# galatolofederico/clip-glass

Measured on AMD Instinct MI355X. Metric: candidate latents scored/sec (GAN→CLIP fitness), StyleGAN2_ffhq_d pop=64, higher is better.
Workload: dtype f16; 1 GPU; StyleGAN2_ffhq_d: StyleGAN2 config-f 1024px G+D + CLIP ViT-B/32, pop=64 per GPU, batch_size=4, n_obj=2; pop_per_gpu=64, global_pop=64, batch_size=4, parallelism=population-shard x1, device=AMD Radeon Graphics (gfx950:sramecc+:xnack-), 256 CUs, hbm_gib=288

## Files before the change

### clip_glass_amd/csrc/kernels.h

```cpp
#pragma once
#include "common.h"

#include <string>
#include <vector>

const char* launch_conv_direct(const ConvParams& p, hipStream_t st);
const char* launch_gemm_direct(const GemmParams& p, hipStream_t st);
const char* launch_conv_tiled(const ConvParams& p, hipStream_t st);
const char* launch_gemm_tiled(const GemmParams& p, hipStream_t st);
const char* launch_conv_stream(const ConvParams& p, hipStream_t st);
const char* launch_conv_gemm(const ConvParams& p, half_t* ws_a, long long cap_a, float* ws_c, long long cap_c, hipStream_t st);
bool conv_stream_applies(const ConvParams& p);
const char* launch_conv_glds(const ConvParams& p, hipStream_t st);
const char* launch_conv_wreg(const ConvParams& p, hipStream_t st);
bool conv_wreg_supported(int Cin, int Cout, int H, int W);
const char* launch_conv_s2(const ConvParams& p, hipStream_t st, bool force = false);
const char* launch_conv_down(const half_t* h, const half_t* xs, const half_t* w1, const half_t* ws, const float* b1, half_t* y,
                             int B, int R, int Cin, int Cout, hipStream_t st);
bool conv_down_supported(int R, int Cin, int Cout);
const char* launch_dblock0(const float* rgb_y, const float* rgb_w, const float* rgb_b, const half_t* w0, const float* b0, const half_t* w1,
                           const half_t* ws, const float* b1, half_t* y, int B, int R, int Cin, int Cout, hipStream_t st, int y_planar8 = 0);
bool dblock0_supported(int R, int Cin, int Cout);
const char* launch_upconv_fused(const ConvParams& p, hipStream_t st);

void launch_pixelnorm(const float* z, float* out, int P, int L, float eps, hipStream_t st);
void launch_dense01_finish(const float* part, int S, long long slab, const float* bias0, const float* w1, const float* b1, float* out, int P, int N,
                           hipStream_t st);
void launch_dense_splitk(const float* x, int ldx, int P, int K, const float* wt, int N, const float* bias, float* out, int ldo,
                         int mode, hipStream_t st);
void launch_dense(const float* x, int ldx, int P, int K, const float* wt, int N, const float* bias,
                  float* out, int ldo, int in_sq, int mode, const float* eps_row, int eps_stride,
                  hipStream_t st);
bool launch_mapping_fused(const float* z, float* out, int P, int L, float eps, const float* const* wt, const float* const* b, int n_layers,
                          hipStream_t st);
struct DenseDesc {
    const float* x; int ldx; int K; const float* wt; int N; const float* bias; float* out; int ldo;
    const float* eps_row; int eps_stride;
};
void launch_dense_multi(const DenseDesc* d_desc, int n_desc, int max_N, int P, int in_sq, int mode, hipStream_t st);
void launch_style_norm(float* s, int ld, int P, int n_layers, const int* d_off, const int* d_len,
                       float* smax, float* eps_row, float eps, hipStream_t st);
void launch_modulate_weights(const half_t* w, long long elems, int Cin, int Cout, const float* sn, int sn_stride,
                              const float* dscale, int ds_stride, int P, half_t* wm, hipStream_t st);
void launch_noise(float* out, int n_mb, int hw, uint32_t layer, uint32_t mb0, uint32_t generation,
                  uint64_t seed, hipStream_t st);

void launch_trgb_tables(const float* wrgb, const float* sn, int sn_stride, const float* smax, int smax_stride, int B, int NT,
                        half_t* tab, hipStream_t st);
void launch_trgb_finish(const float* part, int ntn, int B, int R, const float* bias, const float* yprev, float* yout, hipStream_t st);
bool launch_torgb(const half_t* x, int B, int H, int W, int C, const float* wrgb, const float* bias,
                  const float* sn, int sn_stride, const float* smax, int smax_stride,
                  const float* yprev, float* yout, hipStream_t st);
void launch_finalize_image(const float* y, float* img, long long n, hipStream_t st);
void launch_resize_patches(const float* y, int B, int R, int clip_res, int ps, int ld, half_t* patches,
                           hipStream_t st);
#define GLASS_RESIZE_MAX_TAPS 32
#define PREPROCESS_TY 8
#define PREPROCESS_RB 8
#define PREPROCESS_MAX_R 1024
struct ResizeTaps {
    std::vector<int> start, count;
    std::vector<float> taps;
    std::vector<float> table;
    int max_count = 0, nr = 0, ts = 0;
    size_t lds_bytes = 0;
};
struct ResizeTapsDev {
    const float* table = nullptr;
    int n4 = 0, ts = 0;
    size_t lds_bytes = 0;
};
bool build_resize_taps(int R, int S, int mode, ResizeTaps& t, std::string& why);
void launch_preprocess_patches(const float* y, int B, int R, int clip_res, int ps, int ld, int resize_mode, int normalize,
                               const ResizeTapsDev& t, half_t* patches, hipStream_t st);
void launch_fromrgb(const float* y, int B, int R, int Cout, const float* w, const float* bias,
                    half_t* out, hipStream_t st);
// ... 78 lines not shown
```

### clip_glass_amd/csrc/ops.hip

```cpp
#include <string.h>

#include <string>
#include <vector>

#include "../../include/glass_ops.h"
#include "engine.h"
#include "kernels.h"

namespace {
struct Dev {
    std::vector<void*> ptrs;
    ~Dev() {
        for (void* p : ptrs) hipFree(p);
    }
    template <typename T>
    T* alloc(size_t n) {
        void* q = nullptr;
        if (hipMalloc(&q, (n ? n : 1) * sizeof(T)) != hipSuccess) return nullptr;
        ptrs.push_back(q);
        return (T*)q;
    }
    half_t* up16(const float* src, size_t n) {
        if (!src) return nullptr;
        std::vector<_Float16> h(n);
// ... 63 lines not shown
        std::vector<_Float16> pk2;
        glass_pack_conv(d->w, d->Cout, d->Cin, 3, d->Cin, pk2);
        p.w_up = dv.up16v(pk2);
    }
    p.sn = dv.up32(d->sn, (size_t)d->B * d->Cin); p.sn_stride = d->Cin;
    p.sn16 = dv.up16(d->sn, (size_t)d->B * d->Cin);
    p.dscale = dv.up32(d->dscale, (size_t)d->B * d->Cout); p.ds_stride = d->Cout;
    p.batch_size = d->batch_size > 0 ? d->batch_size : 1;
    p.noise = dv.up32(d->noise, (size_t)(d->B / p.batch_size) * d->Ho * d->Wo);
    p.noise_strength = d->noise_strength;
    p.bias = dv.up32(d->bias, d->Cout);
    p.act = d->act;
    const size_t nout = (size_t)d->B * d->Ho * d->Wo * d->Cout;
    p.res = dv.up16(d->res, nout);
    p.out_scale = d->out_scale;
    half_t* y = dv.alloc<half_t>(nout);
    p.y = y;
    OPREQ(p.x && p.w && y, "device allocation failed");
    if (d->skip_x) {
        OPREQ(d->skip_w && (d->impl == 2 || d->impl == 5), "fused skip branch: impl 2 / 5 with skip_x and skip_w");
        std::vector<_Float16> pks;
        glass_pack_conv(d->skip_w, d->Cout, d->Cin, 1, d->Cin, pks);
        p.skip_w = dv.up16v(pks);
        p.skip_x = dv.up16(d->skip_x, (size_t)d->B * d->Ho * d->Wo * d->Cin);
    }
    half_t* xs_dev = nullptr;
    const size_t nxs = (size_t)d->B * (d->H / 2) * (d->W / 2) * d->Cin;
    if (d->xs_out) {
        OPREQ(d->impl == 2 || d->impl == 5, "blur-down by-product: impl 2 / 5");
        xs_dev = dv.alloc<half_t>(nxs);
        p.xs_out = xs_dev;
    }
    float* yrgb = nullptr;
    const size_t nrgb = (size_t)d->B * 3 * d->Ho * d->Wo;
    if (d->trgb_yout) {
        OPREQ((d->impl == 4 || d->impl == 2 || d->impl == 5) && d->trgb_w && d->trgb_b && d->trgb_sn && d->trgb_smax,
              "fused toRGB: impl 2 / 4 / 5 and all of w / b / sn / smax");
        p.trgb_w = dv.up32(d->trgb_w, 3 * (size_t)d->Cout); p.trgb_b = dv.up32(d->trgb_b, 3);
        p.trgb_sn = dv.up32(d->trgb_sn, (size_t)d->B * d->Cout); p.trgb_sn_stride = d->Cout;
        p.trgb_smax = dv.up32(d->trgb_smax, d->B); p.trgb_smax_stride = 1;
        p.trgb_yprev = dv.up32(d->trgb_yprev, (size_t)d->B * 3 * (d->Ho / 2) * (d->Wo / 2));
        yrgb = dv.alloc<float>(nrgb);
        p.trgb_yout = yrgb;
        if (d->impl == 4) {
            p.y = nullptr;
        } else {
            half_t* tab = dv.alloc<half_t>((size_t)d->B * 32 * d->Cout);
            launch_trgb_tables(p.trgb_w, p.trgb_sn, p.trgb_sn_stride, p.trgb_smax, p.trgb_smax_stride, d->B, d->Cout, tab, 0);
            p.trgb_tab = tab;
        }
    }
    p.x_planar8 = d->x_planar8;
    p.x_planar32 = d->x_planar32;
    if (d->impl == 1) { if (!launch_conv_direct(p, 0)) { glass_set_error("direct conv: unsupported launch"); return GLASS_ERR_ARG; } }
    else if (d->impl == 3) {
        if (!launch_upconv_fused(p, 0)) { glass_set_error("fused up-conv: unsupported shape"); return GLASS_ERR_ARG; }
    } else if (d->impl == 2) {
        if (!launch_conv_tiled(p, 0)) { glass_set_error("tiled conv: unsupported shape"); return GLASS_ERR_ARG; }
    } else if (d->impl == 4) {
        if (!launch_conv_stream(p, 0)) { glass_set_error("streaming conv: unsupported shape"); return GLASS_ERR_ARG; }
    } else if (d->impl == 6) {
        const long long cap_a = (long long)p.Hc * p.Wc * p.KS * p.KS * p.Cin, cap_c = (long long)p.Hc * p.Wc * p.Neff;
        half_t* wa = dv.alloc<half_t>((size_t)(cap_a * p.B));
        float* wc = dv.alloc<float>((size_t)(cap_c * p.B));
        if (!launch_conv_gemm(p, wa, cap_a, wc, cap_c, 0)) { glass_set_error("im2col + GEMM conv: unsupported shape"); return GLASS_ERR_ARG; }
    } else if (d->impl == 5) {
        if (p.skip_x) {
            if (!launch_conv_s2(p, 0, true)) { glass_set_error("LDS-DMA stride-2 conv: unsupported shape"); return GLASS_ERR_ARG; }
        } else if (!launch_conv_glds(p, 0)) { glass_set_error("LDS-DMA conv: unsupported shape"); return GLASS_ERR_ARG; }
    } else if (!(d->up && launch_upconv_fused(p, 0)) && !launch_conv_stream(p, 0) && !launch_conv_tiled(p, 0) && !launch_conv_direct(p, 0)) {
        glass_set_error("no kernel accepts this convolution");
        return GLASS_ERR_ARG;
    }
    int rc = finish();
    if (rc) return rc;
    if (yrgb) {
        GLASS_HIP(hipMemcpy(d->trgb_yout, yrgb, nrgb * sizeof(float), hipMemcpyDeviceToHost));
        return p.y ? down16(d->y, y, nout) : GLASS_OK;
    }
    if (xs_dev && (rc = down16(d->xs_out, xs_dev, nxs))) return rc;
    return down16(d->y, y, nout);
}

extern "C" int glass_op_gemm(int32_t device, int32_t M, int32_t N, int32_t K, const float* a, const float* w,
                             const float* bias, int32_t mode, int32_t impl, float* out) {
    OPREQ(a && w && out && K % 16 == 0, "bad argument");
    GLASS_HIP(hipSetDevice(device));
    Dev dv;
    GemmParams g;
    memset(&g, 0, sizeof g);
    g.a = dv.up16(a, (size_t)M * K); g.w = dv.up16(w, (size_t)N * K); g.M = M; g.N = N; g.K = K;
    g.bias = dv.up32(bias, N); g.mode = mode; g.ldo = N;
    const size_t n = (size_t)M * N;
    half_t* o16 = nullptr; float* o32 = nullptr;
    if (mode <= 1) { o16 = dv.alloc<half_t>(n); g.out16 = o16; }
    else { o32 = mode == 2 ? dv.up32(out, n) : dv.alloc<float>(n); g.out32 = o32; }
    if (impl == 1) launch_gemm_direct(g, 0);
    else if (impl == 2) {
        if (!launch_gemm_tiled(g, 0)) { glass_set_error("tiled gemm: unsupported shape"); return GLASS_ERR_ARG; }
    } else if (!launch_gemm_tiled(g, 0)) launch_gemm_direct(g, 0);
    int rc = finish();
    if (rc) return rc;
    if (o16) return down16(out, o16, n);
    GLASS_HIP(hipMemcpy(out, o32, n * sizeof(float), hipMemcpyDeviceToHost));
    return GLASS_OK;
}

extern "C" int glass_op_dense(int32_t device, int32_t P, int32_t K, int32_t N, const float* x, const float* wt,
                              const float* bias, int32_t in_sq, int32_t mode, const float* eps_row, float* out) {
// ... 462 lines not shown
```

### clip_glass_amd/csrc/upfir.hip

```cpp
#include "common.h"
#include "kernels.h"
#include <algorithm>
#include <mutex>
#include <vector>

#define ROWB 80

struct UpGeo {
    int NTn, ngroups;
    int tiles_x, n_seg, S;
    int NXI, NYI, n_grids;
    int WT;
    unsigned invPX, invPY;
    unsigned inv2PX, inv2PY;
};

namespace {
constexpr int U_PH = 9, U_PW = 33;
constexpr int U_NVB = 9 * 32 * 4, U_NB = (U_NVB + 255) / 256;
constexpr int U_A_BYTES = ((U_PH * U_PW * ROWB + 15) / 16) * 16;
struct UStep {
    static constexpr int RW = 2, MR = 4 * RW, TR = 2 * MR, PH = MR + 1;
    static constexpr int NVA = PH * U_PW * 4, NA = (NVA + 255) / 256;
    static constexpr int A_BYTES = ((PH * U_PW * ROWB + 15) / 16) * 16;
    static constexpr int T_BYTES = TR * 64 * 64;
    static constexpr int STAGE = A_BYTES + 9 * 32 * ROWB;
    static constexpr int R0 = ((T_BYTES > STAGE ? T_BYTES : STAGE) + 1023) / 1024 * 1024;
    static constexpr int OFF_LNZ = R0;
    static constexpr int OFF_HS = OFF_LNZ + TR * 60 * 4;
    static constexpr int LDS = OFF_HS + 256 * 48;
};
constexpr int U_OFF_STY = 46848;
constexpr int U_OFF_DS = U_OFF_STY + 8 * 1024;
constexpr int U_OFF_PS = U_OFF_DS + 8 * 128;
constexpr int U_OFF_BI = U_OFF_PS + 8 * 64;
constexpr int U_OFF_NZ = U_OFF_BI + 128;
static_assert(UStep::LDS == 81664 && 2 * UStep::LDS <= 163840, "two workgroups per CU");
static_assert(U_OFF_NZ + 16 * 60 * 4 <= 65536 && U_OFF_STY >= U_A_BYTES + 9 * 32 * ROWB && UStep::A_BYTES == U_A_BYTES, "constant tables fit behind the staging images");
__device__ __forceinline__ int u_opaque(int v) { asm volatile("" : "+v"(v)); return v; }
__device__ __forceinline__ int u_stage_row(int r) { return (r & ~7) | ((r & 7) >> 1) | ((r & 1) << 2); }
__device__ __forceinline__ int u_tpos(int x) { return (x & 1) * 32 + (x >> 1); }
__device__ __forceinline__ int u_fir_col(int ci) { return ci ^ (((ci >> 2) ^ (ci >> 1)) & 1); }
}

template <bool GRID>
__global__ __launch_bounds__(256, 2) void upfir2_kernel(ConvParams p, UpGeo g) {
    using US = UStep;
    constexpr int RW = US::RW, MR = US::MR, TR = US::TR;
    constexpr int PW = U_PW, NA = US::NA, NVB = U_NVB, NB = U_NB, A_BYTES = US::A_BYTES;
    constexpr int U_OFF_LNZ = US::OFF_LNZ, U_OFF_HS = US::OFF_HS;
    extern __shared__ __attribute__((aligned(16))) char smem[];
    char* As = smem;
    char* Bs = smem + A_BYTES;
    half_t* T = (half_t*)smem;

    const int id = blockIdx.x;
// ... 367 lines not shown
                    const int ltx = oxl + 1 + jx;
                    tr[jx] = (const char*)T + u_tpos(ltx) * 64 + ((cg ^ ((ltx >> 2) & 3)) * 16);
                }
                const long long rowpitch = (long long)p.Wo * (p.y_planar8 ? 8 : p.Cout);
                half_t* yp = p.y_planar8 ? p.y + ((((long long)img0 * 4 * g.NTn + (n0 >> 3) + cg) * p.Ho + ovy0) * p.Wo + ox) * 8
                                          : p.y + (((long long)img0 * p.Ho + ovy0) * p.Wo + ox) * p.Cout + n0 + cg * 8;
                h8 cv[4];
                float cnz;
                auto rdrow = [&](int r, h8 (&v_)[4], float& nz_) {
#pragma unroll
                    for (int jx = 0; jx < 4; ++jx) v_[jx] = *(const h8*)(tr[jx] + r * 4096);
                    nz_ = *(const float*)(smem + U_OFF_LNZ + (r * 60 + oxl) * 4);
                };
                rdrow(0, cv, cnz);
#pragma unroll
                for (int r = 0; r < TR; ++r) {
                    h8 nv[4];
                    float nnz;
                    if (r + 1 < TR) rdrow(r + 1, nv, nnz);
                    __builtin_amdgcn_sched_barrier(0);
                    hs[r & 3] = (cv[1] + cv[2]) * f3 + (cv[0] + cv[3]);
                    const h8 bn = bias8 + (half_t)cnz;
                    h8 v = (hs[(r - 3) & 3] + hs[r & 3]) * fq4 + ((hs[(r - 2) & 3] + hs[(r - 1) & 3]) * ft4 + bn);
                    v = __builtin_elementwise_max(v, v * slope) * kps;
                    if ((step > 0 || r >= 4) && ovy0 + r < p.Ho) *(h8*)yp = v;
                    yp += rowpitch;
                    __builtin_amdgcn_sched_barrier(0);
                    if (r + 1 < TR) {
#pragma unroll
                        for (int jx = 0; jx < 4; ++jx) cv[jx] = nv[jx];
                        cnz = nnz;
                    }
                }
                *(h8*)(hs_slot) = hs[1]; *(h8*)(hs_slot + 16) = hs[2]; *(h8*)(hs_slot + 32) = hs[3];
            }
            if (step + 1 < g.S && Y0 + TR * (step + 1) - 4 < out_rows) {
                const int my0n = my0 + MR;
                const bool plain_n = mx0 >= 1 && my0n >= 1 && my0n + MR - 1 < p.H && mx0 + 31 < p.W;
                load_b(0);
                if (plain && plain_n) {
                    const int dstep = MR * p.W * p.Cin;
#pragma unroll
                    for (int k = 0; k < NA; ++k) a_goff[k] += dstep;
                } else {
                    aim(my0n, 0);
                }
                load_a(0);
                have = true;
            }
        }
    }
}

static unsigned u_inv(int d) { return (unsigned)((0x100000000ULL + (unsigned)d - 1) / (unsigned)d); }

static int upfir2_model_steps(int per_seg, int out_rows, int TR, int slots, int fallback) {
    struct Key { int per_seg, out_rows, slots, S; };
    static std::mutex mu;
    static std::vector<Key> cache;
    std::lock_guard<std::mutex> lk(mu);
    for (const Key& k : cache)
        if (k.per_seg == per_seg && k.out_rows == out_rows && k.slots == slots) return k.S;
    int best = fallback;
    double best_t = 1e30;
    std::vector<double> heap;
    for (int S = 1; S <= 16; ++S) {
        const int R = (TR - 4) + TR * (S - 1);
        if (R > out_rows + TR - 1 && S > 1) break;
        const int n_seg = (out_rows + R - 1) / R;
        if ((long long)per_seg * n_seg < slots) break;
        heap.assign(slots, 0.0);
        auto cmp = [](double a, double b) { return a > b; };
        for (int seg = 0; seg < n_seg; ++seg) {
            int steps = 0;
            for (int st = 0; st < S; ++st) {
                if (seg * R + (st ? TR * st - 4 : 0) >= out_rows) break;
                ++steps;
            }
            for (int w = 0; w < per_seg; ++w) {
                std::pop_heap(heap.begin(), heap.end(), cmp);
                heap.back() += steps + 0.5;
                std::push_heap(heap.begin(), heap.end(), cmp);
            }
        }
        double t = 0;
        for (double v : heap) t = v > t ? v : t;
        if (t < best_t - 1e-9) { best_t = t; best = S; }
    }
    cache.push_back({per_seg, out_rows, slots, best});
    return best;
}

static const char* launch_upfir2(const ConvParams& p, hipStream_t st) {
    if (p.Cin > 512 || p.H < 8 || p.W < 8) return nullptr;
    if ((long long)p.B * p.H * p.W * p.Cin >= (1LL << 31) || 9LL * p.Cout * p.Cin >= (1LL << 31)) return nullptr;
    if (p.x_bstride != (long long)p.H * p.W * p.Cin) return nullptr;
    const bool lean = p.w_bstride && !p.sn16 && !p.dscale;
    if (p.y_planar8 && !lean) return nullptr;
    constexpr int LDS = UStep::LDS, TR = UStep::TR;
    if (!glass_lds_fits(LDS)) return nullptr;
    static DevOnce once;
    once.run([&] {
        (void)hipFuncSetAttribute((const void*)upfir2_kernel<true>, hipFuncAttributeMaxDynamicSharedMemorySize, LDS);
        (void)hipFuncSetAttribute((const void*)upfir2_kernel<false>, hipFuncAttributeMaxDynamicSharedMemorySize, LDS);
    });
    UpGeo g;
    g.NTn = p.Cout / 32;
    if (p.w_bstride) { g.NXI = 1; g.NYI = 1; }
    else {
        const int nxi_max = p.W + 1 >= 11 ? 8 : 3;
        g.NXI = p.B < nxi_max ? p.B : nxi_max;
        g.NYI = (p.B + g.NXI - 1) / g.NXI;
        if (g.NYI > 8) g.NYI = 8;
    }
    g.n_grids = (p.B + g.NXI * g.NYI - 1) / (g.NXI * g.NYI);
    const int PX = p.W + 1, PY = p.H + 1;
    g.tiles_x = (2 * PX * g.NXI - 2 + 59) / 60;
    const int out_rows = 2 * PY * g.NYI - 2;
    int S = 16;
    for (; S > 1; --S) {
        const int R = (TR - 4) + TR * (S - 1);
        const long long wgs = (long long)g.n_grids * g.tiles_x * ((out_rows + R - 1) / R) * g.NTn;
        if (wgs >= (S > 8 ? 5120 : 2048) && R <= out_rows + TR - 1) break;
    }
    if (!lean && S <= 2) S = upfir2_model_steps(g.n_grids * g.tiles_x * g.NTn, out_rows, TR, 2 * glass_cu_count(), S);
    g.S = S;
    const int R = (TR - 4) + TR * (S - 1);
    g.n_seg = (out_rows + R - 1) / R;
    g.WT = g.n_grids * g.n_seg * g.tiles_x;
    int ng = 1;
    if (!p.w_bstride) {
        const long long per_tile = 9LL * 32 * p.Cin * 2;
        while (ng < 8 && g.NTn % (ng * 2) == 0 && (g.NTn / ng) * per_tile > (1200LL << 10)) ng *= 2;
    }
    g.ngroups = ng;
    g.invPX = u_inv(PX); g.invPY = u_inv(PY); g.inv2PX = u_inv(2 * PX); g.inv2PY = u_inv(2 * PY);
    const char* name = lean ? "upfir2_kernel<false>" : "upfir2_kernel<true>";
    if (p.dry_run) return name;
    const int Pp = 8 / ng;
    const int grid = 8 * ((g.WT + Pp - 1) / Pp) * (g.NTn / ng);
    if (lean) hipLaunchKernelGGL((upfir2_kernel<false>), dim3(grid), dim3(256), LDS, st, p, g);
    else hipLaunchKernelGGL((upfir2_kernel<true>), dim3(grid), dim3(256), LDS, st, p, g);
    return name;
}

const char* launch_upconv_fused(const ConvParams& p, hipStream_t st) {
    if (!p.up || !p.w_up || p.y32 || !p.y || p.res || (p.sn && !p.sn16)) return nullptr;
    if (p.Cin % 32 != 0 || p.Cout % 32 != 0 || p.KS != 3) return nullptr;
    if (p.x_planar8 || p.x_planar32) return nullptr;
    return launch_upfir2(p, st);
}
```

### clip_glass_amd/ops.py

```python
import ctypes as C

import numpy as np

from .engine import _check, _f32, _fp, load_library


class ConvDesc(C.Structure):
    _fields_ = [("B", C.c_int32), ("H", C.c_int32), ("W", C.c_int32), ("Cin", C.c_int32), ("Cout", C.c_int32),
                ("KS", C.c_int32), ("stride", C.c_int32), ("pad", C.c_int32), ("up", C.c_int32),
                ("Ho", C.c_int32), ("Wo", C.c_int32), ("broadcast_x", C.c_int32), ("act", C.c_int32),
                ("batch_size", C.c_int32), ("impl", C.c_int32),
                ("noise_strength", C.c_float), ("out_scale", C.c_float),
                ("x", C.POINTER(C.c_float)), ("w", C.POINTER(C.c_float)), ("sn", C.POINTER(C.c_float)),
                ("dscale", C.POINTER(C.c_float)), ("noise", C.POINTER(C.c_float)), ("bias", C.POINTER(C.c_float)),
                ("res", C.POINTER(C.c_float)), ("y", C.POINTER(C.c_float)),
                ("trgb_w", C.POINTER(C.c_float)), ("trgb_b", C.POINTER(C.c_float)), ("trgb_sn", C.POINTER(C.c_float)),
                ("trgb_smax", C.POINTER(C.c_float)), ("trgb_yprev", C.POINTER(C.c_float)),
                ("trgb_yout", C.POINTER(C.c_float)),
                ("skip_x", C.POINTER(C.c_float)), ("skip_w", C.POINTER(C.c_float)), ("xs_out", C.POINTER(C.c_float)),
                ("x_planar8", C.c_int32), ("x_planar32", C.c_int32)]


def to_planar8(a):
    B, H, W, Cc = a.shape
    return np.ascontiguousarray(a.reshape(B, H, W, Cc // 8, 8).transpose(0, 3, 1, 2, 4))


def to_planar32(a):
    B, H, W, Cc = a.shape
    return np.ascontiguousarray(a.reshape(B, H, W, Cc // 32, 32).transpose(0, 3, 1, 2, 4))


def from_planar32(a, B, H, W, Cc):
    return np.ascontiguousarray(a.reshape(B, Cc // 32, H, W, 32).transpose(0, 2, 3, 1, 4)).reshape(B, H, W, Cc)


def from_planar8(a, B, H, W, Cc):
    return np.ascontiguousarray(a.reshape(B, Cc // 8, H, W, 8).transpose(0, 2, 3, 1, 4)).reshape(B, H, W, Cc)


def _opt(a):
    if a is None:
        return None, None
    a = _f32(a)
    return a, _fp(a)


def conv(x, w, *, stride=1, pad=None, up=False, sn=None, dscale=None, noise=None, noise_strength=0.0,
         batch_size=1, bias=None, act=False, res=None, out_scale=1.0, impl=0, broadcast_x=False, B=None, device=0,
         torgb=None, skip=None, xs_out=None, planar_x=False, both=False, planar32_x=False):
    lib = load_library()
    x = _f32(x); w = _f32(w)
    Bx, H, W, Cin = x.shape
    if planar_x:
        x = to_planar8(x)
    if planar32_x:
        x = to_planar32(x)
    B = B if B is not None else Bx
    Cout, _, KS, _ = w.shape
    pad = (KS // 2) if pad is None else pad
    if up:
        Ho, Wo = 2 * H, 2 * W
    else:
        Ho, Wo = (H + 2 * pad - KS) // stride + 1, (W + 2 * pad - KS) // stride + 1
    y = np.empty((B, Ho, Wo, Cout), dtype=np.float32)
    d = ConvDesc()
    d.B, d.H, d.W, d.Cin, d.Cout = B, H, W, Cin, Cout
    d.KS, d.stride, d.pad, d.up, d.Ho, d.Wo = KS, stride, pad, int(up), Ho, Wo
    d.broadcast_x, d.act, d.batch_size, d.impl = int(broadcast_x), int(act), batch_size, impl
    d.noise_strength, d.out_scale = noise_strength, out_scale
    d.x_planar8 = int(planar_x)
    d.x_planar32 = int(planar32_x)
    keep = []
    d.x, d.w, d.y = _fp(x), _fp(w), _fp(y)
    for name, val in (("sn", sn), ("dscale", dscale), ("noise", noise), ("bias", bias), ("res", res)):
        a, p = _opt(val)
        keep.append(a)
        if p is not None:
            setattr(d, name, p)
    if skip is not None:
        for name, val in zip(("skip_x", "skip_w"), skip):
            a, p = _opt(val)
            keep.append(a)
            setattr(d, name, p)
    if xs_out is not None:
        d.xs_out = _fp(xs_out)
    yrgb = None
    if torgb is not None:
        yrgb = np.empty((B, 3, Ho, Wo), dtype=np.float32)
        for name in ("w", "b", "sn", "smax", "yprev"):
            a, p = _opt(torgb.get(name))
            keep.append(a)
            if p is not None:
                setattr(d, "trgb_" + name, p)
        d.trgb_yout = _fp(yrgb)
    lib.glass_op_conv.argtypes = [C.c_int32, C.POINTER(ConvDesc)]
    _check(lib, lib.glass_op_conv(device, C.byref(d)))
    if both:
        return yrgb, y
    return yrgb if yrgb is not None else y


def gemm(a, w, bias=None, mode=3, impl=0, acc=None, device=0):
    lib = load_library()
    a = _f32(a); w = _f32(w)
    M, K = a.shape
    N = w.shape[0]
    out = _f32(acc).copy() if acc is not None else np.empty((M, N), dtype=np.float32)
    b, bp = _opt(bias)
    lib.glass_op_gemm.argtypes = [C.c_int32] * 4 + [C.POINTER(C.c_float)] * 3 + [C.c_int32, C.c_int32, C.POINTER(C.c_float)]
    _check(lib, lib.glass_op_gemm(device, M, N, K, _fp(a), _fp(w), bp, mode, impl, _fp(out)))
    return out


def dense(x, wt, bias=None, in_sq=False, mode=0, eps_row=None, device=0):
    lib = load_library()
    x = _f32(x); wt = _f32(wt)
    P, K = x.shape
    N = wt.shape[1]
    out = np.empty((P, N), dtype=np.float32)
    b, bp = _opt(bias)
    e, ep = _opt(eps_row)
    fp = C.POINTER(C.c_float)
    lib.glass_op_dense.argtypes = [C.c_int32] * 4 + [fp, fp, fp, C.c_int32, C.c_int32, fp, fp]
    _check(lib, lib.glass_op_dense(device, P, K, N, _fp(x), _fp(wt), bp, int(in_sq), mode, ep, _fp(out)))
    return out


# ... 268 lines not shown
```

### include/glass_ops.h

```cpp
#ifndef GLASS_OPS_H
#define GLASS_OPS_H
#include <stdint.h>
#ifdef __cplusplus
extern "C" {
#endif

typedef struct glass_conv_desc {
    int32_t B, H, W, Cin, Cout;
    int32_t KS, stride, pad;
    int32_t up;
    int32_t Ho, Wo;
    int32_t broadcast_x;
    int32_t act;
    int32_t batch_size;
    int32_t impl;
    float noise_strength, out_scale;
    const float* x;
    const float* w;
    const float* sn;
    const float* dscale;
    const float* noise;
    const float* bias;
    const float* res;
    float* y;
    const float* trgb_w;
    const float* trgb_b;
    const float* trgb_sn;
    const float* trgb_smax;
    const float* trgb_yprev;
    float* trgb_yout;
    const float* skip_x;
    const float* skip_w;
    float* xs_out;
    int32_t x_planar8;
    int32_t x_planar32;
} glass_conv_desc;

int glass_op_conv(int32_t device, const glass_conv_desc* d);
int glass_op_gemm(int32_t device, int32_t M, int32_t N, int32_t K, const float* a, const float* w,
                  const float* bias, int32_t mode, int32_t impl, float* out);
int glass_op_dense(int32_t device, int32_t P, int32_t K, int32_t N, const float* x, const float* wt ,
                   const float* bias, int32_t in_sq, int32_t mode, const float* eps_row, float* out);
int glass_op_torgb(int32_t device, int32_t B, int32_t H, int32_t C, const float* x, const float* wrgb ,
                   const float* bias, const float* sn, const float* smax, const float* yprev, float* yout);
int glass_op_blur(int32_t device, int32_t mode , int32_t B, int32_t H, int32_t C,
                  const float* x, float* out);
int glass_op_dblock_down(int32_t device, int32_t B, int32_t R, int32_t Cin, int32_t Cout, const float* h, const float* x,
                         const float* w1, const float* wskip, const float* b1, float* y);
int glass_op_dblock0(int32_t device, int32_t B, int32_t R, int32_t impl, const float* y, const float* frgb_w, const float* frgb_b,
                     const float* w0, const float* b0, const float* w1, const float* wskip, const float* b1, float* out);
int glass_op_fromrgb(int32_t device, int32_t B, int32_t R, int32_t Cout, const float* y ,
                     const float* w , const float* bias, float* out );
int glass_op_mbstd(int32_t device, int32_t B, int32_t hw, int32_t C, int32_t Cpad, int32_t batch_size, int32_t group,
                   const float* x, float* out);
int glass_op_resize(int32_t device, int32_t B, int32_t R, int32_t S, int32_t ps, const float* y ,
                    float* patches );
int glass_op_preprocess(int32_t device, int32_t B, int32_t R, int32_t S, int32_t ps, int32_t resize_mode, int32_t normalize,
                        const float* y , float* patches );
int glass_op_layernorm(int32_t device, int32_t M, int32_t D, const float* x, const float* g, const float* b, float* out);
int glass_op_attention(int32_t device, int32_t n_img, int32_t L, int32_t heads, int32_t causal, const float* qkv,
                       float* out);
int glass_op_noise(int32_t device, int32_t n_mb, int32_t hw, uint32_t layer, uint32_t mb0, uint32_t generation,
                   uint64_t seed, float* out);
int glass_op_gpt2_sample(int32_t device, int32_t rows, int32_t V, const float* logits, float temperature, int32_t top_k,
                         uint64_t seed, int32_t generation, int32_t first_row, int32_t step, int32_t purpose, int32_t* out);
int glass_op_gpt2_gemm(int32_t device, int32_t form, int32_t M, int32_t N, int32_t K, int32_t lda, int32_t mode, int32_t width,
                       const float* a, const float* w, const float* bias, const float* lng, const float* lnb, const float* pst_in,
                       int32_t np_in, float* out, float* stats_out, float* pst_out, int32_t* splits);
int glass_op_gpt2_attention(int32_t device, int32_t form, int32_t P, int32_t nd, int32_t past, int32_t Tmax, int32_t heads, int32_t S,
                            const float* qkv, const float* bias, float* kc, float* vc, float* out);
int glass_op_gpt2_head(int32_t device, int32_t M, int32_t V, int32_t K, int32_t tail, const float* x, const float* wte, const float* lng,
                       const float* lnb, const float* wpe, int32_t npos, int32_t past, int32_t step, float* logits, float* pair_val,
                       int32_t* pair_idx, int32_t* token, float* stats, float* x_next, float* stats_next, int32_t* state);
int glass_op_gpt2_embed_step(int32_t device, int32_t M, int32_t V, int32_t K, const int32_t* token, const float* wte, const float* wpe,
                             int32_t npos, int32_t past, int32_t step, float* x, float* stats);
int glass_op_mfma_probe(int32_t device, const float* a , const float* b , float* d );

int glass_host_pack_conv(const float* w, int32_t Cout, int32_t Cin, int32_t KS, int32_t up, float* out);
int glass_host_resize_taps(int32_t R, int32_t S, int32_t mode, int32_t* start, int32_t* count, float* taps, int32_t max);

#ifdef __cplusplus
}
#endif
#endif
```

Baseline: 2244 candidates/s.

## Add wide 512-thread fused upsample-conv kernel with taller row tiles

Adds a new upfir2w kernel for the fused transposed-conv + FIR upsample. It uses 512 threads (8 waves), twice the output rows per step and a larger LDS footprint, and the launcher selects it by default when weights are shared and H>=32. The taller tiles are meant to raise reuse of the staged weights and cut halo overhead per workgroup, and the step-count model is re-tuned for one workgroup per CU. A post_scale parameter is also threaded through the op API, and impl 7 forces the old narrow kernel. The trade-off is lower occupancy from the larger LDS use.

```diff
diff --git a/clip_glass_amd/csrc/kernels.h b/clip_glass_amd/csrc/kernels.h
--- a/clip_glass_amd/csrc/kernels.h
+++ b/clip_glass_amd/csrc/kernels.h
@@ -21,7 +21,7 @@
 const char* launch_dblock0(const float* rgb_y, const float* rgb_w, const float* rgb_b, const half_t* w0, const float* b0, const half_t* w1,
                            const half_t* ws, const float* b1, half_t* y, int B, int R, int Cin, int Cout, hipStream_t st, int y_planar8 = 0);
 bool dblock0_supported(int R, int Cin, int Cout);
-const char* launch_upconv_fused(const ConvParams& p, hipStream_t st);
+const char* launch_upconv_fused(const ConvParams& p, hipStream_t st, bool narrow = false);
 
 void launch_pixelnorm(const float* z, float* out, int P, int L, float eps, hipStream_t st);
 void launch_dense01_finish(const float* part, int S, long long slab, const float* bias0, const float* w1, const float* b1, float* out, int P, int N,
diff --git a/clip_glass_amd/csrc/ops.hip b/clip_glass_amd/csrc/ops.hip
--- a/clip_glass_amd/csrc/ops.hip
+++ b/clip_glass_amd/csrc/ops.hip
@@ -139,9 +139,13 @@
     }
     p.x_planar8 = d->x_planar8;
     p.x_planar32 = d->x_planar32;
+    if (d->post_scale) {
+        OPREQ(d->impl == 3 || d->impl == 7, "post_scale: the fused up-conv only (impl 3 / 7)");
+        p.post_scale16 = dv.up16(d->post_scale, (size_t)d->B * d->Cout); p.post_stride = d->Cout;
+    }
     if (d->impl == 1) { if (!launch_conv_direct(p, 0)) { glass_set_error("direct conv: unsupported launch"); return GLASS_ERR_ARG; } }
-    else if (d->impl == 3) {
-        if (!launch_upconv_fused(p, 0)) { glass_set_error("fused up-conv: unsupported shape"); return GLASS_ERR_ARG; }
+    else if (d->impl == 3 || d->impl == 7) {
+        if (!launch_upconv_fused(p, 0, d->impl == 7)) { glass_set_error("fused up-conv: unsupported shape"); return GLASS_ERR_ARG; }
     } else if (d->impl == 2) {
         if (!launch_conv_tiled(p, 0)) { glass_set_error("tiled conv: unsupported shape"); return GLASS_ERR_ARG; }
     } else if (d->impl == 4) {
diff --git a/clip_glass_amd/csrc/upfir.hip b/clip_glass_amd/csrc/upfir.hip
--- a/clip_glass_amd/csrc/upfir.hip
+++ b/clip_glass_amd/csrc/upfir.hip
@@ -2,6 +2,7 @@
 #include "kernels.h"
 #include <algorithm>
 #include <mutex>
+#include <type_traits>
 #include <vector>
 
 #define ROWB 80
@@ -475,15 +476,336 @@
     }
 }
 
+namespace {
+struct WStep {
+    static constexpr int RW = 2, NWV = 8, MR = NWV * RW, TR = 2 * MR, PH = MR + 1;
+    static constexpr int A_ROWS = PH * U_PW, B_ROWS = 9 * 32, ROWS = A_ROWS + B_ROWS;
+    static constexpr int NV = ROWS * 4, NR = (NV + 511) / 512;
+    static constexpr int NRA = (A_ROWS * 4 + 511) / 512;
+    static constexpr int T_MIX = A_ROWS * 4 - (NRA - 1) * 512;
+    static constexpr int T_END = NV - (NR - 1) * 512;
+    static constexpr int STAGE = ROWS * 64;
+    static constexpr int T_BYTES = TR * 64 * 64;
+    static constexpr int OFF_STY = 2 * STAGE;
+    static constexpr int OFF_DS = OFF_STY + 8 * 1024;
+    static constexpr int OFF_PS = OFF_DS + 8 * 128;
+    static constexpr int OFF_BI = OFF_PS + 8 * 64;
+    static constexpr int OFF_NZ = OFF_BI + 128;
+    static constexpr int OFF_HS = T_BYTES;
+    static constexpr int LDS = OFF_HS + 2 * 256 * 48;
+};
+static_assert(WStep::NR == 7 && WStep::NRA == 5 && WStep::T_MIX == 196 && WStep::T_END == 324, "staging rounds");
+static_assert(WStep::OFF_NZ + WStep::TR * 60 * 4 <= WStep::T_BYTES && WStep::LDS <= 163840, "tables under the T tile, one workgroup per CU");
+__device__ __forceinline__ int swz(int row, int chunk) { return (row << 6) + ((chunk ^ ((row >> 2) & 3)) << 4); }
+}
+
+__global__ __launch_bounds__(512) void upfir2w_kernel(ConvParams p, UpGeo g) {
+    using WS = WStep;
+    constexpr int RW = WS::RW, MR = WS::MR, TR = WS::TR, PW = U_PW, NR = WS::NR, NRA = WS::NRA;
+    extern __shared__ __attribute__((aligned(16))) char smem[];
+    half_t* T = (half_t*)smem;
+
+    const int id = blockIdx.x;
+    const int xcd = id & 7, rest = id >> 3;
+    const int G = g.ngroups, NTg = g.NTn / G, Pp = 8 / G;
+    const int nt = (xcd % G) * NTg + rest % NTg;
+    const int wt = (rest / NTg) * Pp + xcd / G;
+    if (wt >= g.WT) return;
+    const int txi = wt % g.tiles_x, seg = (wt / g.tiles_x) % g.n_seg, gi = wt / (g.tiles_x * g.n_seg);
+    const int n0 = nt * 32;
+    const int img0 = gi * g.NXI * g.NYI;
+    const int PX = p.W + 1, PY = p.H + 1;
+    const int mx0 = txi * 30 - 1;
+    const int Y0 = seg * ((TR - 4) + TR * (g.S - 1));
+    const int out_rows = 2 * PY * g.NYI - 2;
+    const int ixi0 = (int)__umulhi((unsigned)max(mx0 - 1, 0), g.invPX);
+
+    int a_goff[NRA];
+    int okm = 0, selm = 0;
+    h8 rv[NR];
+    for (int step = 0; step < g.S; ++step) {
+        const int o_first = Y0 + (step ? TR * step - 4 : 0);
+        if (o_first >= out_rows) break;
+        const int my0 = (Y0 >> 1) - 1 + MR * step;
+        const int iyi0 = (int)__umulhi((unsigned)max(my0 - 1, 0), g.invPY);
+        auto sel_img = [&](int sel) {
+            const int iyi = min(iyi0 + (sel >> 2), g.NYI - 1), ixi = min(ixi0 + (sel & 3), g.NXI - 1);
+            return min(img0 + iyi * g.NXI + ixi, p.B - 1);
+        };
+        auto w_goff = [&](int k) {
+            const int t = u_opaque(threadIdx.x);
+            const int wr = min(max((t >> 2) + 128 * k - WS::A_ROWS, 0), WS::B_ROWS - 1);
+            return ((wr >> 5) * p.Cout + n0 + (wr & 31)) * p.Cin + (t & 3) * 8;
+        };
+        auto load_k = [&](int k, int c0) {
+            if (k < NRA - 1) rv[k] = *(const h8*)(p.x + a_goff[k] + c0);
+            else if (k == NRA - 1) rv[k] = *(const h8*)((threadIdx.x >= WS::T_MIX ? p.w_up + w_goff(k) : p.x + a_goff[k]) + c0);
+            else rv[k] = *(const h8*)(p.w_up + w_goff(k) + c0);
+        };
+        auto store_k = [&](int k, char* buf, int c0) {
+            const int t = threadIdx.x, part = t & 3;
+            char* sb = buf + swz(t >> 2, part) + k * (128 * 64);
+            if (k < NRA) {
+                const h8 zero = {0, 0, 0, 0, 0, 0, 0, 0};
+                h8 a = ((okm >> k) & 1) ? rv[k] : zero;
+                a = a * *(const h8*)(smem + WS::OFF_STY + (c0 + part * 8) * 2 + ((selm >> (3 * k)) & 7) * 1024);
+                if (k == NRA - 1 && t >= WS::T_MIX) a = rv[k];
+                *(h8*)sb = a;
+            } else if (k < NR - 1 || t < WS::T_END) {
+                *(h8*)sb = rv[k];
+            }
+        };
+
+        __syncthreads();
+        {
+            okm = 0;
+            selm = 0;
+            const int t = u_opaque(threadIdx.x), part = t & 3;
+#pragma unroll
+            for (int k = 0; k < NRA; ++k) {
+                const int pix = (t >> 2) + 128 * k;
+                const int pr = pix / PW, pc = pix - pr * PW;
+                const int vy = my0 - 1 + pr, vx = mx0 - 1 + pc;
+                const int iyi = (int)__umulhi((unsigned)max(vy, 0), g.invPY), ixi = (int)__umulhi((unsigned)max(vx, 0), g.invPX);
+                const int iy = vy - iyi * PY, ix = vx - ixi * PX;
+                const int img = img0 + iyi * g.NXI + ixi;
+                const bool ok = pix < WS::A_ROWS && vy >= 0 && vx >= 0 && iy < p.H && ix < p.W && iyi < g.NYI && ixi < g.NXI && img < p.B;
+                a_goff[k] = ok ? img * (int)p.x_bstride + (iy * p.W + ix) * p.Cin + part * 8 : part * 8;
+                okm |= (ok ? 1 : 0) << k;
+                selm |= ((((iyi - iyi0) << 2) + (ixi - ixi0)) & 7) << (3 * k);
+            }
+        }
+        {
+            const int t = u_opaque(threadIdx.x);
+            const int cin8 = p.Cin >> 3;
+            h8 sv;
+#pragma unroll
+            for (int j = 0; j < 8; ++j) sv[j] = (half_t)1.f;
+            float dsv = 1.f, biv = 0.f, nzv4[4];
+            half_t psv = (half_t)1.f;
+            if (p.sn16) {
+                const int e = min(t, 8 * cin8 - 1);
+                const int sel = e / cin8, piece = e - sel * cin8;
+                sv = *(const h8*)(p.sn16 + (long long)sel_img(sel) * p.sn_stride + piece * 8);
+            }
+            const int sel = (t >> 5) & 7, ch = t & 31;
+            if (p.dscale) dsv = p.dscale[(long long)sel_img(sel) * p.ds_stride + n0 + ch];
+            if (p.post_scale16) psv = p.post_scale16[(long long)sel_img(sel) * p.post_stride + n0 + ch];
+            if (p.bias && t < 32) biv = p.bias[n0 + t];
+#pragma unroll
+            for (int u = 0; u < 4; ++u) {
+                nzv4[u] = 0.f;
+                if (p.noise) {
+                    const int e = min(t + 512 * u, TR * 60 - 1);
+                    const int r = e / 60, c = e - r * 60;
+                    const int ovy = max(Y0 + TR * step + r - 4, 0), ovx = txi * 60 + c;
+                    const int iyi = (int)__umulhi((unsigned)ovy, g.inv2PY), ixi = (int)__umulhi((unsigned)ovx, g.inv2PX);
+                    const int oy = min(ovy - iyi * 2 * PY, p.Ho - 1), ox = min(ovx - ixi * 2 * PX, p.Wo - 1);
+                    const int img = min(img0 + min(iyi, g.NYI - 1) * g.NXI + min(ixi, g.NXI - 1), p.B - 1);
+                    nzv4[u] = p.noise[((long long)(img / p.batch_size) * p.Ho + oy) * p.Wo + ox];
+                }
+            }
+#pragma unroll
+            for (int k = 0; k < NR; ++k) load_k(k, 0);
+            if (t < 8 * cin8) {
+                const int sel = t / cin8, piece = t - sel * cin8;
+                *(h8*)(smem + WS::OFF_STY + sel * 1024 + piece * 16) = sv;
+            }
+            if (t < 256) {
+                *(float*)(smem + WS::OFF_DS + t * 4) = dsv;
+                *(half_t*)(smem + WS::OFF_PS + t * 2) = psv;
+            }
+            if (t < 32) *(float*)(smem + WS::OFF_BI + t * 4) = biv;
+#pragma unroll
+            for (int u = 0; u < 4; ++u)
+                if (t + 512 * u < TR * 60) *(float*)(smem + WS::OFF_NZ + (t + 512 * u) * 4) = p.noise_strength * nzv4[u];
+            __syncthreads();
+        }
+
+        f16x acc[RW][4];
+#pragma unroll
+        for (int i = 0; i < RW; ++i)
+#pragma unroll
+            for (int j = 0; j < 4; ++j)
+#pragma unroll
+                for (int q = 0; q < 16; ++q) acc[i][j][q] = 0.f;
+        auto mfma_block = [&](const char* buf, auto&& between) {
+            const int tm = u_opaque(threadIdx.x), lr = tm & 31, kh = (tm >> 5) & 1, wave = tm >> 6;
+            __builtin_amdgcn_s_setprio(1);
+#pragma unroll
+            for (int kk = 0; kk < 2; ++kk) {
+#pragma unroll
+                for (int ay = 0; ay < 2; ++ay) {
+#pragma unroll
+                    for (int ax = 0; ax < 2; ++ax) {
+                        h8 wf[2][2];
+#pragma unroll
+                        for (int ky = ay * 2; ky < (ay ? 3 : 2); ++ky)
+#pragma unroll
+                            for (int kx = ax * 2; kx < (ax ? 3 : 2); ++kx)
+                                wf[ky & 1][kx & 1] = *(const h8*)(buf + swz(WS::A_ROWS + (ky * 3 + kx) * 32 + lr, kk * 2 + kh));
+#pragma unroll
+                        for (int i = 0; i < RW; ++i) {
+                            const int prow = wave * RW + i + 1 - ay;
+                            const h8 xf = *(const h8*)(buf + swz(prow * PW + lr + 1 - ax, kk * 2 + kh));
+#pragma unroll
+                            for (int ky = ay * 2; ky < (ay ? 3 : 2); ++ky)
+#pragma unroll
+                                for (int kx = ax * 2; kx < (ax ? 3 : 2); ++kx)
+                                    acc[i][(ky & 1) * 2 + (kx & 1)] = mfma32(wf[ky & 1][kx & 1], xf, acc[i][(ky & 1) * 2 + (kx & 1)]);
+                        }
+                        __builtin_amdgcn_sched_barrier(0);
+                        between(kk * 4 + ay * 2 + ax);
+                        __builtin_amdgcn_sched_barrier(0);
+                    }
+                }
+            }
+            __builtin_amdgcn_s_setprio(0);
+        };
+        const int n_stages = p.Cin >> 5;
+#pragma unroll
+        for (int k = 0; k < NR; ++k) store_k(k, smem, 0);
+        if (n_stages > 1) {
+#pragma unroll
+            for (int k = 0; k < NR; ++k) load_k(k, 32);
+        }
+        auto stage = [&](int s, auto mode) {
+            asm volatile("s_waitcnt lgkmcnt(0)" ::: "memory");
+            __builtin_amdgcn_s_barrier();
+            const char* cur = smem + (s & 1) * WS::STAGE;
+            char* nxt = smem + ((s + 1) & 1) * WS::STAGE;
+            mfma_block(cur, [&](int j) {
+                if (j < NR) {
+                    if (decltype(mode)::value >= 1) store_k(j, nxt, (s + 1) * 32);
+                    if (decltype(mode)::value >= 2) load_k(j, (s + 2) * 32);
+                }
+            });
+        };
+        for (int s = 0; s < n_stages - 2; ++s) stage(s, std::integral_constant<int, 2>());
+        for (int s = max(n_stages - 2, 0); s < n_stages - 1; ++s) stage(s, std::integral_constant<int, 1>());
+        stage(n_stages - 1, std::integral_constant<int, 0>());
+
+        const int ovy0 = Y0 + TR * step - 4;
+        const int t = u_opaque(threadIdx.x), lane = t & 63, wave = t >> 6, lr = lane & 31, kh = lane >> 5;
+        const int gr = t >> 8, tl = t & 255;
+        const int cg = tl & 3, oxl = u_fir_col(tl >> 2);
+        f4 dq[RW][4];
+        {
+            const int ixl = (int)__umulhi((unsigned)max(mx0 + lr, 0), g.invPX) - ixi0;
+#pragma unroll
+            for (int i = 0; i < RW; ++i) {
+                const int iyl = (int)__umulhi((unsigned)max(my0 + RW * wave + i, 0), g.invPY) - iyi0;
+                const char* dp = smem + WS::OFF_DS + (((iyl << 2) + ixl) & 7) * 128 + kh * 16;
+#pragma unroll
+                for (int gq = 0; gq < 4; ++gq) dq[i][gq] = *(const f4*)(dp + gq * 32);
+            }
+        }
+        const int ovx = txi * 60 + min(oxl, 59);
+        const int ixo = (int)__umulhi((unsigned)ovx, g.inv2PX);
+        const int ox = ovx - ixo * 2 * PX;
+        const bool col_on = tl < 240 && ox < p.Wo && ixo < g.NXI;
+        h8 bias8, psa, psb;
+        {
+            const f4 b0 = *(const f4*)(smem + WS::OFF_BI + cg * 32), b1 = *(const f4*)(smem + WS::OFF_BI + cg * 32 + 16);
+#pragma unroll
+            for (int j = 0; j < 4; ++j) { bias8[j] = (half_t)b0[j]; bias8[j + 4] = (half_t)b1[j]; }
+            const int sx = (ixo - ixi0) & 3;
+            psa = *(const h8*)(smem + WS::OFF_PS + sx * 64 + cg * 16);
+            psb = *(const h8*)(smem + WS::OFF_PS + (4 + sx) * 64 + cg * 16);
+        }
+        float nzr[TR / 2];
+#pragma unroll
+        for (int r = 0; r < TR / 2; ++r) nzr[r] = *(const float*)(smem + WS::OFF_NZ + ((gr * (TR / 2) + r) * 60 + min(oxl, 59)) * 4);
+        __syncthreads();
+
+        {
+            char* tw = (char*)T + ((2 * wave * RW) * 64 + lr) * 64 + kh * 8;
+            int so[4];
+#pragma unroll
+            for (int gq = 0; gq < 4; ++gq) so[gq] = (gq ^ ((lr >> 1) & 3)) * 16;
+#pragma unroll
+            for (int i = 0; i < RW; ++i)
+#pragma unroll
+                for (int ph = 0; ph < 4; ++ph)
+#pragma unroll
+                    for (int gq = 0; gq < 4; ++gq) {
+                        h4 o;
+#pragma unroll
+                        for (int q = 0; q < 4; ++q) o[q] = (half_t)(acc[i][ph][gq * 4 + q] * dq[i][gq][q]);
+                        *(h4*)(tw + so[gq] + ((2 * i + (ph >> 1)) * 64 + (ph & 1) * 32) * 64) = o;
+                    }
+        }
+        __syncthreads();
+
+        if (col_on) {
+            char* slot_in = smem + WS::OFF_HS + (((step + 1) & 1) * 256 + tl) * 48;
+            char* slot_out = smem + WS::OFF_HS + ((step & 1) * 256 + tl) * 48;
+            h8 hs[4];
+            const half_t f3 = (half_t)3.f, fq4 = (half_t)0.0625f, ft4 = (half_t)0.1875f;
+            const half_t slope = (half_t)(p.act ? 0.2f : 1.f);
+            const half_t gain = (half_t)((p.act ? GLASS_SQRT2 : 1.f) * p.out_scale);
+            const h8 kpsa = psa * gain, kpsb = psb * gain;
+            const char* tr[4];
+#pragma unroll
+            for (int jx = 0; jx < 4; ++jx) {
+                const int ltx = oxl + 1 + jx;
+                tr[jx] = (const char*)T + gr * (TR / 2) * 4096 + u_tpos(ltx) * 64 + ((cg ^ ((ltx >> 2) & 3)) * 16);
+            }
+            if (gr == 0) {
+                hs[1] = *(const h8*)(slot_in); hs[2] = *(const h8*)(slot_in + 16); hs[3] = *(const h8*)(slot_in + 32);
+            } else {
+#pragma unroll
+                for (int q = 1; q < 4; ++q) {
+                    h8 wv[4];
+#pragma unroll
+                    for (int jx = 0; jx < 4; ++jx) wv[jx] = *(const h8*)(tr[jx] + (q - 4) * 4096);
+                    hs[q] = (wv[1] + wv[2]) * f3 + (wv[0] + wv[3]);
+                }
+            }
+            const int yb = 2 * PY * (iyi0 + 1);
+            h8 cv[4];
+#pragma unroll
+            for (int jx = 0; jx < 4; ++jx) cv[jx] = *(const h8*)(tr[jx]);
+#pragma unroll
+            for (int r = 0; r < TR / 2; ++r) {
+                h8 nv[4];
+                if (r + 1 < TR / 2) {
+#pragma unroll
+                    for (int jx = 0; jx < 4; ++jx) nv[jx] = *(const h8*)(tr[jx] + (r + 1) * 4096);
+                }
+                __builtin_amdgcn_sched_barrier(0);
+                hs[r & 3] = (cv[1] + cv[2]) * f3 + (cv[0] + cv[3]);
+                const int tr_row = gr * (TR / 2) + r;
+                const int ovy = ovy0 + tr_row;
+                const bool second = ovy >= yb;
+                const int iyo = iyi0 + (second ? 1 : 0);
+                const int oy = ovy - 2 * PY * iyo;
+                const int img = img0 + iyo * g.NXI + ixo;
+                const bool emit = (step > 0 || tr_row >= 4) && oy >= 0 && oy < p.Ho && iyo < g.NYI && img < p.B;
+                const h8 bn = bias8 + (half_t)nzr[r];
+                const h8 v = (hs[(r - 3) & 3] + hs[r & 3]) * fq4 + ((hs[(r - 2) & 3] + hs[(r - 1) & 3]) * ft4 + bn);
+                half_t* yp = p.y + (((long long)img * p.Ho + oy) * p.Wo + ox) * p.Cout + n0 + cg * 8;
+                if (emit) *(h8*)yp = __builtin_elementwise_max(v, v * slope) * (second ? kpsb : kpsa);
+                __builtin_amdgcn_sched_barrier(0);
+                if (r + 1 < TR / 2) {
+#pragma unroll
+                    for (int jx = 0; jx < 4; ++jx) cv[jx] = nv[jx];
+                }
+            }
+            if (gr == 1) { *(h8*)(slot_out) = hs[1]; *(h8*)(slot_out + 16) = hs[2]; *(h8*)(slot_out + 32) = hs[3]; }
+        }
+    }
+}
+
 static unsigned u_inv(int d) { return (unsigned)((0x100000000ULL + (unsigned)d - 1) / (unsigned)d); }
 
 static int upfir2_model_steps(int per_seg, int out_rows, int TR, int slots, int fallback) {
-    struct Key { int per_seg, out_rows, slots, S; };
+    struct Key { int per_seg, out_rows, slots, TR, S; };
     static std::mutex mu;
     static std::vector<Key> cache;
     std::lock_guard<std::mutex> lk(mu);
     for (const Key& k : cache)
-        if (k.per_seg == per_seg && k.out_rows == out_rows && k.slots == slots) return k.S;
+        if (k.per_seg == per_seg && k.out_rows == out_rows && k.slots == slots && k.TR == TR) return k.S;
     int best = fallback;
     double best_t = 1e30;
     std::vector<double> heap;
@@ -510,22 +832,25 @@
         for (double v : heap) t = v > t ? v : t;
         if (t < best_t - 1e-9) { best_t = t; best = S; }
     }
-    cache.push_back({per_seg, out_rows, slots, best});
+    cache.push_back({per_seg, out_rows, slots, TR, best});
     return best;
 }
 
-static const char* launch_upfir2(const ConvParams& p, hipStream_t st) {
+static const char* launch_upfir2(const ConvParams& p, hipStream_t st, bool narrow) {
     if (p.Cin > 512 || p.H < 8 || p.W < 8) return nullptr;
     if ((long long)p.B * p.H * p.W * p.Cin >= (1LL << 31) || 9LL * p.Cout * p.Cin >= (1LL << 31)) return nullptr;
     if (p.x_bstride != (long long)p.H * p.W * p.Cin) return nullptr;
     const bool lean = p.w_bstride && !p.sn16 && !p.dscale;
     if (p.y_planar8 && !lean) return nullptr;
-    constexpr int LDS = UStep::LDS, TR = UStep::TR;
+    constexpr int LDS = UStep::LDS;
     if (!glass_lds_fits(LDS)) return nullptr;
+    const bool wide = !narrow && !p.w_bstride && p.H >= 32 && glass_lds_fits(WStep::LDS);
+    const int TR = wide ? WStep::TR : UStep::TR;
     static DevOnce once;
     once.run([&] {
         (void)hipFuncSetAttribute((const void*)upfir2_kernel<true>, hipFuncAttributeMaxDynamicSharedMemorySize, LDS);
         (void)hipFuncSetAttribute((const void*)upfir2_kernel<false>, hipFuncAttributeMaxDynamicSharedMemorySize, LDS);
+        (void)hipFuncSetAttribute((const void*)upfir2w_kernel, hipFuncAttributeMaxDynamicSharedMemorySize, WStep::LDS);
     });
     UpGeo g;
     g.NTn = p.Cout / 32;
@@ -546,7 +871,13 @@
         const long long wgs = (long long)g.n_grids * g.tiles_x * ((out_rows + R - 1) / R) * g.NTn;
         if (wgs >= (S > 8 ? 5120 : 2048) && R <= out_rows + TR - 1) break;
     }
-    if (!lean && S <= 2) S = upfir2_model_steps(g.n_grids * g.tiles_x * g.NTn, out_rows, TR, 2 * glass_cu_count(), S);
+    if (!wide) {
+        if (!lean && S <= 2) S = upfir2_model_steps(g.n_grids * g.tiles_x * g.NTn, out_rows, TR, 2 * glass_cu_count(), S);
+    } else if (S <= 1) {
+        const int per_seg = g.n_grids * g.tiles_x * g.NTn;
+        if ((long long)per_seg * ((out_rows + (TR - 4) - 1) / (TR - 4)) < glass_cu_count()) S = 2 * TR - 4 <= out_rows + TR - 1 ? 2 : 1;
+        else S = upfir2_model_steps(per_seg, out_rows, TR, glass_cu_count(), S);
+    }
     g.S = S;
     const int R = (TR - 4) + TR * (S - 1);
     g.n_seg = (out_rows + R - 1) / R;
@@ -558,18 +889,19 @@
     }
     g.ngroups = ng;
     g.invPX = u_inv(PX); g.invPY = u_inv(PY); g.inv2PX = u_inv(2 * PX); g.inv2PY = u_inv(2 * PY);
-    const char* name = lean ? "upfir2_kernel<false>" : "upfir2_kernel<true>";
+    const char* name = wide ? "upfir2w_kernel" : lean ? "upfir2_kernel<false>" : "upfir2_kernel<true>";
     if (p.dry_run) return name;
     const int Pp = 8 / ng;
     const int grid = 8 * ((g.WT + Pp - 1) / Pp) * (g.NTn / ng);
-    if (lean) hipLaunchKernelGGL((upfir2_kernel<false>), dim3(grid), dim3(256), LDS, st, p, g);
+    if (wide) hipLaunchKernelGGL(upfir2w_kernel, dim3(grid), dim3(512), WStep::LDS, st, p, g);
+    else if (lean) hipLaunchKernelGGL((upfir2_kernel<false>), dim3(grid), dim3(256), LDS, st, p, g);
     else hipLaunchKernelGGL((upfir2_kernel<true>), dim3(grid), dim3(256), LDS, st, p, g);
     return name;
 }
 
-const char* launch_upconv_fused(const ConvParams& p, hipStream_t st) {
+const char* launch_upconv_fused(const ConvParams& p, hipStream_t st, bool narrow) {
     if (!p.up || !p.w_up || p.y32 || !p.y || p.res || (p.sn && !p.sn16)) return nullptr;
     if (p.Cin % 32 != 0 || p.Cout % 32 != 0 || p.KS != 3) return nullptr;
     if (p.x_planar8 || p.x_planar32) return nullptr;
-    return launch_upfir2(p, st);
+    return launch_upfir2(p, st, narrow);
 }
diff --git a/clip_glass_amd/ops.py b/clip_glass_amd/ops.py
--- a/clip_glass_amd/ops.py
+++ b/clip_glass_amd/ops.py
@@ -18,7 +18,7 @@
                 ("trgb_smax", C.POINTER(C.c_float)), ("trgb_yprev", C.POINTER(C.c_float)),
                 ("trgb_yout", C.POINTER(C.c_float)),
                 ("skip_x", C.POINTER(C.c_float)), ("skip_w", C.POINTER(C.c_float)), ("xs_out", C.POINTER(C.c_float)),
-                ("x_planar8", C.c_int32), ("x_planar32", C.c_int32)]
+                ("x_planar8", C.c_int32), ("x_planar32", C.c_int32), ("post_scale", C.POINTER(C.c_float))]
 
 
 def to_planar8(a):
@@ -48,7 +48,7 @@
 
 def conv(x, w, *, stride=1, pad=None, up=False, sn=None, dscale=None, noise=None, noise_strength=0.0,
          batch_size=1, bias=None, act=False, res=None, out_scale=1.0, impl=0, broadcast_x=False, B=None, device=0,
-         torgb=None, skip=None, xs_out=None, planar_x=False, both=False, planar32_x=False):
+         torgb=None, skip=None, xs_out=None, planar_x=False, both=False, planar32_x=False, post_scale=None):
     lib = load_library()
     x = _f32(x); w = _f32(w)
     Bx, H, W, Cin = x.shape
@@ -73,7 +73,7 @@
     d.x_planar32 = int(planar32_x)
     keep = []
     d.x, d.w, d.y = _fp(x), _fp(w), _fp(y)
-    for name, val in (("sn", sn), ("dscale", dscale), ("noise", noise), ("bias", bias), ("res", res)):
+    for name, val in (("sn", sn), ("dscale", dscale), ("noise", noise), ("bias", bias), ("res", res), ("post_scale", post_scale)):
         a, p = _opt(val)
         keep.append(a)
         if p is not None:
diff --git a/include/glass_ops.h b/include/glass_ops.h
--- a/include/glass_ops.h
+++ b/include/glass_ops.h
@@ -34,6 +34,7 @@
     float* xs_out;
     int32_t x_planar8;
     int32_t x_planar32;
+    const float* post_scale;
 } glass_conv_desc;
 
 int glass_op_conv(int32_t device, const glass_conv_desc* d);
```

Result: no change. 2231 candidates/s (-0.6%).
